# wwood/CoverM

Measured on NVIDIA H100. Metric: reads/sec `coverm contig` (mean+trimmed_mean+covered_fraction), higher is better.
Workload: dtype i32

## Files before the change

coverm_b200/csrc/cmb_k2.cuh:

```cuda
#pragma once
#include "cmb_k2_slots.cuh"

struct K2Args {
  const uint32_t* off_span;
  const uint32_t* len;
  const uint32_t* chunk_first;
  const int32_t* carry_in;
  cmb_contig_stats* rows;
  uint32_t tid_begin, n_local, n_chunks, excl;
  int32_t* arena;
  const uint32_t* word_off;
  const uint16_t* buckets;
  uint32_t* span_bits;
  uint32_t* load_stats;
  const uint64_t* bin_base;
  uint32_t* bins;
  uint64_t pool_cap;
  uint32_t* bin_hi;
  uint32_t* error_flags;
};

#ifndef CMB_K2_DENSE_SPANS
#define CMB_K2_DENSE_SPANS 160
#endif
constexpr uint32_t K2_DENSE_SPANS = CMB_K2_DENSE_SPANS;
static_assert(K2_STAGES >= 2, "a round's rows are requested one round before it is reduced");
static_assert(K2_CHUNK_SPANS == CHUNK_SPANS && K2_WARPS == 8, "a chunk is 8 bitmap words of 32 spans");

constexpr uint32_t K2_ROUND = 32;
constexpr uint32_t K2_BUF_BYTES = K2_ROUND * 128;
constexpr uint32_t K2_BOX_ROWS = K2_ROUND;
constexpr uint32_t K2_STAGE_CODES = 1024;
constexpr uint32_t K2_STAGE_BYTES = K2_STAGE_CODES * 2;
template <bool BUCKETS>
__host__ __device__ constexpr uint32_t k2_warp_bytes() { return BUCKETS ? K2_BUF_BYTES + K2_STAGES * K2_STAGE_BYTES : K2_STAGES * K2_BUF_BYTES; }
constexpr uint32_t K2_SMEM_MISC = K2_WARPS * K2_STAGES * 8  +
                                  K2_WARPS * 128 ;
template <bool BUCKETS>
__host__ __device__ constexpr uint32_t k2_smem_bytes() { return K2_WARPS * k2_warp_bytes<BUCKETS>() + K2_SMEM_MISC; }
static_assert(k2_warp_bytes<true>() % 1024 == 0 && k2_warp_bytes<false>() % 1024 == 0, "round buffers are whole swizzle atoms");

__device__ __forceinline__ uint32_t k2_rounds(uint32_t pop, bool dense) { return dense ? CHUNK_SPANS / K2_ROUND : (pop + K2_ROUND - 1) / K2_ROUND; }

template <bool HIST, bool CLEAN, bool BUCKETS>
__global__ void __launch_bounds__(K2_THREADS, CMB_K2_MINBLOCKS) k2_scan_reduce(const __grid_constant__ CUtensorMap tmap, const K2Args a) {
  extern __shared__ __align__(1024) uint8_t smem[];
  const uint32_t lane = threadIdx.x & 31, warp = threadIdx.x >> 5;
  constexpr uint32_t RING = K2_WARPS * k2_warp_bytes<BUCKETS>();
  uint8_t* ring = smem + warp * k2_warp_bytes<BUCKETS>();
  uint64_t* bars = reinterpret_cast<uint64_t*>(smem + RING) + warp * K2_STAGES;
  uint32_t* words = reinterpret_cast<uint32_t*>(smem + RING + K2_WARPS * K2_STAGES * 8) + warp * 32;
  uint32_t(&fw)[8] = *reinterpret_cast<uint32_t(*)[8]>(words);
  uint32_t(&w)[8] = *reinterpret_cast<uint32_t(*)[8]>(words + 8);
  uint32_t* wo = words + 16;

  const bool hist = HIST && __ldg(a.bin_base + a.n_local) <= a.pool_cap;
  if (HIST && !hist && blockIdx.x == 0 && threadIdx.x == 0) atomicOr(a.error_flags, ERR_CAPACITY);

  const uint32_t W = gridDim.x * K2_WARPS, g = blockIdx.x * K2_WARPS + warp;
  auto load_word = [&](uint32_t ck) -> uint32_t { return ck < a.n_chunks && lane < K2_WARPS ? a.span_bits[ck * K2_WARPS + lane] : 0u; };
  auto load_off = [&](uint32_t ck) -> uint32_t { return BUCKETS && ck < a.n_chunks && lane <= K2_WARPS ? __ldg(a.word_off + ck * K2_WARPS + lane) : 0u; };
  auto spread = [&](uint32_t word, uint32_t* to, uint32_t off = 0, uint32_t* to_off = nullptr) -> uint32_t {
    __syncwarp();
    if (lane < K2_WARPS) to[lane] = word;
    if (to_off && lane <= K2_WARPS) to_off[lane] = off;
    __syncwarp();
    return __reduce_add_sync(FULL, __popc(word));
  };

  if (lane == 0) {
    for (uint32_t s = 0; s < K2_STAGES; ++s) mbar_init(smem_u32(bars + s), 1);
    fence_barrier_init();
  }
  if (BUCKETS)
    for (uint32_t u = lane; u < K2_BUF_BYTES / 16; u += 32) reinterpret_cast<int4*>(ring)[u] = make_int4(0, 0, 0, 0);
  __syncwarp();

  uint32_t fk = g, fr = 0, fpop = 0;
  bool fdense = false;
  uint32_t f_word = load_word(fk);
  uint32_t f_off = load_off(fk), fo = 0;
  uint32_t n_loaded = 0, n_dense = 0, n_events = 0;
  auto f_enter = [&]() {
    for (; fk < a.n_chunks; fk += W) {
      const uint32_t word = f_word;
      f_word = load_word(fk + W);
      fo = f_off;
      f_off = load_off(fk + W);
      fpop = spread(word, fw);
      fdense = fpop >= K2_DENSE_SPANS;
      fr = 0;
      if (k2_rounds(fpop, fdense)) {
        n_loaded += fdense ? CHUNK_SPANS : fpop;
        n_dense += fdense;
        return;
      }
    }
  };
  auto fill = [&](uint32_t fi) {
    if (fk < a.n_chunks) {
      uint8_t* buf = ring + (fi % K2_STAGES) * K2_BUF_BYTES;
      const uint32_t bar = smem_u32(bars + fi % K2_STAGES);
      if constexpr (BUCKETS) {
        uint32_t wf, wl;
        k2_round_words(fw, fdense ? CHUNK_SPANS : fpop, fdense, fr, wf, wl);
        const uint32_t b0 = __shfl_sync(FULL, fo, wf), b1 = __shfl_sync(FULL, fo, wl + 1);
        const uint32_t base = b0 & ~7u, units = min((b1 - base + 7) / 8, K2_STAGE_CODES / 8);
        uint8_t* stg = ring + K2_BUF_BYTES + (fi % K2_STAGES) * K2_STAGE_BYTES;
        const int4* src = reinterpret_cast<const int4*>(a.buckets + base);
        for (uint32_t u = lane; u < units; u += 32) cp_async_16(smem_u32(stg + u * 16), src + u);
        n_events += b1 - b0;
      } else if (fdense) {
        if (lane == 0) {
          fence_proxy_async_smem();
          mbar_arrive_expect_tx(bar, K2_BUF_BYTES);
          tma_load_2d(smem_u32(buf), &tmap, 0, (int32_t)(fk * CHUNK_ROWS + fr * K2_BOX_ROWS), bar);
        }
      } else {
        const uint32_t n = min(K2_ROUND, fpop - fr * K2_ROUND);
        const uint32_t sp = k2_slot_span(fw, fr * K2_ROUND + lane, false);
        const uint32_t q = lane >> 3, unit = lane & 7;
        const int4* src = reinterpret_cast<const int4*>(a.arena + (uint64_t)fk * CHUNK) + unit;
        for (uint32_t r0 = 0; r0 < n; r0 += 4) {
          const uint32_t row = r0 + q;
          const uint32_t rsp = __shfl_sync(FULL, sp, row & 31);
          if (row < n) cp_async_16(smem_u32(buf + row * 128 + ((unit ^ (row & 7)) << 4)), src + rsp * (SPAN / 4));
        }
        if (lane == 0) mbar_arrive(bar);
      }
      if (++fr == k2_rounds(fpop, fdense)) {
        fk += W;
        f_enter();
      }
    }
    cp_async_commit();
  };
  f_enter();
  for (uint32_t p = 0; p + 1 < K2_STAGES; ++p) fill(p);

  const uint32_t E = a.excl;
  auto flush = [&](uint32_t c, uint32_t sf, uint32_t sw, uint64_t sd, uint32_t top) {
    cmb_contig_stats* rowp = a.rows + a.tid_begin + c;
    if (sf) atomicAdd((unsigned long long*)&rowp->covered_full, (unsigned long long)sf);
    if (sw) atomicAdd((unsigned long long*)&rowp->covered_window, (unsigned long long)sw);
    if (sd) atomicAdd((unsigned long long*)&rowp->sum_depth_window, (unsigned long long)sd);
    if (top) atomicMax(a.bin_hi + c, top);
  };
  auto bin_add = [&](uint64_t bin0, uint64_t bin1, int depth, uint32_t cnt, uint32_t& top) {
    if (depth < 0 || (uint64_t)depth >= bin1 - bin0) {
      atomicOr(a.error_flags, ERR_INTERNAL);
      return;
    }
    atomicAdd(a.bins + bin0 + (uint32_t)depth, cnt);
    top = max(top, (uint32_t)depth);
  };

  uint32_t c_word = load_word(g), c_off = load_off(g);
  uint32_t n_cf = 0, n_cl = 0;
  int n_cin = 0;
  if (g < a.n_chunks) {
    n_cf = __ldg(a.chunk_first + g);
    n_cl = __ldg(a.chunk_first + g + 1);
    n_cin = __ldg(a.carry_in + g);
  }
  uint32_t i = 0;
  for (uint32_t k = g; k < a.n_chunks; k += W) {
    const uint32_t word = c_word, off = c_off, cf = n_cf, cl = n_cl;
    const int cin = n_cin;
    c_word = load_word(k + W);
    c_off = load_off(k + W);
    if (k + W < a.n_chunks) {
      n_cf = __ldg(a.chunk_first + k + W);
      n_cl = __ldg(a.chunk_first + k + W + 1);
      n_cin = __ldg(a.carry_in + k + W);
    }
    const uint32_t pop = spread(word, w, off, BUCKETS ? wo : nullptr);
    const bool dense = pop >= K2_DENSE_SPANS;
    const uint32_t nr = k2_rounds(pop, dense), nslots = dense ? CHUNK_SPANS : pop;
    const uint32_t span0 = k * CHUNK_SPANS;
    uint32_t pc = cf, c_first = 0xffffffffu;
    int pd = cin;
    for (uint32_t r = 0; r < nr; ++r, ++i) {
      __syncwarp();
      fill(i + K2_STAGES - 1);
      const uint32_t j = r * K2_ROUND + lane;
      const bool valid = j < nslots;
      const uint32_t s = k2_slot_span(w, j, dense), sn = k2_slot_span(w, j + 1, dense);
      uint32_t c = 0xffffffffu, cstart = 0;
      K2Win win{0u, 0u, 0u};
      uint64_t bin0 = 0, bin1 = 0;
      if (valid) {
        uint32_t lo = cf, hi = cl;
        while (lo < hi) {
          const uint32_t mid = (lo + hi + 1) >> 1;
          if (__ldg(a.off_span + mid) <= span0 + s) lo = mid;
          else hi = mid - 1;
        }
        c = lo;
        cstart = __ldg(a.off_span + c);
        win = k2_window(__ldg(a.len + c), E);
        if (hist) {
          bin0 = __ldg(a.bin_base + c);
          bin1 = __ldg(a.bin_base + c + 1);
        }
      }
      const uint32_t st = i % K2_STAGES;
      if (!BUCKETS) mbar_wait(smem_u32(bars + st), (i / K2_STAGES) & 1);
      cp_async_wait<K2_STAGES - 1>();
      __syncwarp();
      uint8_t* rows = BUCKETS ? ring : ring + st * K2_BUF_BYTES;
      if (BUCKETS) {
        const uint32_t wf = __shfl_sync(FULL, s, 0) / 32, wl = __shfl_sync(FULL, s, min(nslots - r * K2_ROUND, K2_ROUND) - 1) / 32;
        const uint32_t base = wo[wf] & ~7u;
        const uint16_t* stg = reinterpret_cast<const uint16_t*>(ring + K2_BUF_BYTES + st * K2_STAGE_BYTES);
        k2_round_events(
            w, wo, dense, r, wf, wl, lane, 32,
            [&](uint32_t p) { return p - base < K2_STAGE_CODES ? (uint32_t)stg[p - base] : (uint32_t)__ldg(a.buckets + p); },
            [&](uint32_t rw, uint32_t e, int d) {
              atomicAdd(reinterpret_cast<int*>(rows + rw * 128 + (((e >> 2) ^ (rw & 7)) << 4) + ((e & 3) << 2)), d);
            });
        __syncwarp();
      }
      uint8_t* row = rows + lane * 128;
      int total = 0;
      uint32_t ev = 0;
      if (valid) {
#pragma unroll
        for (uint32_t u = 0; u < SPAN / 4; ++u) {
          const int4 v = *reinterpret_cast<const int4*>(row + ((u ^ (lane & 7)) << 4));
          const uint32_t e4 = (v.x != 0 ? 1u : 0u) | (v.y != 0 ? 2u : 0u) | (v.z != 0 ? 4u : 0u) | (v.w != 0 ? 8u : 0u);
          total += (v.x + v.y) + (v.z + v.w);
          ev |= e4 << (4 * u);
          if constexpr (!BUCKETS && CLEAN)
            if (e4) reinterpret_cast<int4*>(a.arena + (uint64_t)(span0 + s) * SPAN)[u] = make_int4(0, 0, 0, 0);
        }
      }
      int incl = total;
#pragma unroll
      for (uint32_t d = 1; d < 32; d <<= 1) {
        const int ov = __shfl_up_sync(FULL, incl, d);
        const uint32_t oc = __shfl_up_sync(FULL, c, d);
        if (lane >= d && oc == c) incl += ov;
      }
      const int depth = incl - total + (c == pc ? pd : 0);
      const uint32_t rel = (span0 + s - cstart) * SPAN;
      const uint32_t from = j == 0 && c == cf ? (span0 - cstart) * SPAN : rel;
      const uint32_t to = rel + (sn - s) * SPAN;
      K2Acc acc{0u, 0u, 0ull};
      uint32_t top = 0;
      int out = 0;
      if (valid)
        out = k2_slot_runs(
            acc, win, depth, ev, rel, from, to,
            [&](uint32_t e) { return *reinterpret_cast<const int*>(row + (((e >> 2) ^ (lane & 7)) << 4) + ((e & 3) << 2)); },
            [&](int d, uint32_t n) {
              if (hist) bin_add(bin0, bin1, d, n, top);
            });
      if (BUCKETS)
#pragma unroll
        for (uint32_t u = 0; u < SPAN / 4; ++u)
          if (ev >> (4 * u) & 15u) *reinterpret_cast<int4*>(row + ((u ^ (lane & 7)) << 4)) = make_int4(0, 0, 0, 0);
      pc = __shfl_sync(FULL, c, 31);
      pd = __shfl_sync(FULL, out, 31);
      if (r == 0) c_first = __shfl_sync(FULL, c, 0);
      uint32_t sf = acc.cov_full, sw = acc.cov_win;
      uint64_t sd = acc.sum_win;
#pragma unroll
      for (uint32_t d = 1; d < 32; d <<= 1) {
        const uint32_t of = __shfl_down_sync(FULL, sf, d), ow = __shfl_down_sync(FULL, sw, d);
        const uint64_t od = __shfl_down_sync(FULL, sd, d);
        const uint32_t ot = HIST ? __shfl_down_sync(FULL, top, d) : 0u;
        const uint32_t oc = __shfl_down_sync(FULL, c, d);
        if (lane + d < 32 && oc == c) {
          sf += of;
          sw += ow;
          sd += od;
          top = max(top, ot);
        }
      }
      const uint32_t prev_c = __shfl_up_sync(FULL, c, 1);
      if (valid && (lane == 0 || prev_c != c)) flush(c, sf, sw, sd, top);
    }
    if (lane == 0 && cin != 0 && c_first != cf) {
      const uint32_t cstart = __ldg(a.off_span + cf);
      const K2Win win = k2_window(__ldg(a.len + cf), E);
      const uint32_t s0 = k2_slot_span(w, 0, dense);
      K2Acc acc{0u, 0u, 0ull};
      uint32_t top = 0;
      const uint32_t nw = k2_close_run(acc, win, cin, (span0 - cstart) * SPAN, (span0 + s0 - cstart) * SPAN);
      if (hist && nw) bin_add(__ldg(a.bin_base + cf), __ldg(a.bin_base + cf + 1), cin, nw, top);
      flush(cf, acc.cov_full, acc.cov_win, acc.sum_win, top);
    }
    if (CLEAN && word) a.span_bits[k * K2_WARPS + lane] = 0;
  }
  if (lane == 0 && n_loaded) {
    atomicAdd(a.load_stats + 0, n_loaded);
    atomicAdd(a.load_stats + 1, n_dense);
    if (BUCKETS) atomicAdd(a.load_stats + 2, n_events);
  }
}
```

coverm_b200/csrc/cmb_k2_slots.cuh:

```cuda
#pragma once
#include <stdint.h>

#ifdef __CUDACC__
#define K2_HD __host__ __device__ __forceinline__
#else
#define K2_HD inline
#endif

constexpr uint32_t K2_CHUNK_SPANS = 256;

K2_HD uint32_t k2_popc(uint32_t x) {
#ifdef __CUDA_ARCH__
  return __popc(x);
#else
  return (uint32_t)__builtin_popcount(x);
#endif
}

K2_HD uint32_t k2_low_bit(uint32_t x) {
#ifdef __CUDA_ARCH__
  return (uint32_t)__ffs((int)x) - 1u;
#else
  return (uint32_t)__builtin_ctz(x);
#endif
}

K2_HD uint32_t k2_nth_bit(uint32_t x, uint32_t n) {
  uint32_t pos = 0;
#pragma unroll
  for (uint32_t w = 16; w; w >>= 1) {
    const uint32_t lo = k2_popc(x & ((1u << w) - 1u));
    if (n >= lo) {
      n -= lo;
      x >>= w;
      pos += w;
    }
  }
  return pos;
}

K2_HD uint32_t k2_slot_span(const uint32_t (&w)[8], uint32_t j, bool dense) {
  if (dense) return j < K2_CHUNK_SPANS ? j : K2_CHUNK_SPANS;
  uint32_t base = 0, word = 0, rem = j;
  bool found = false;
#pragma unroll
  for (uint32_t q = 0; q < 8; ++q) {
    const uint32_t p = k2_popc(w[q]);
    if (!found) {
      if (rem < p) {
        found = true;
        base = 32 * q;
        word = w[q];
      } else {
        rem -= p;
      }
    }
  }
  return found ? base + k2_nth_bit(word, rem) : K2_CHUNK_SPANS;
}


K2_HD void k2_round_words(const uint32_t (&w)[8], uint32_t nslots, bool dense, uint32_t r, uint32_t& wf, uint32_t& wl) {
  const uint32_t j1 = r * 32 + 31 < nslots ? r * 32 + 31 : nslots - 1;
  wf = k2_slot_span(w, r * 32, dense) / 32;
  wl = k2_slot_span(w, j1, dense) / 32;
}

K2_HD uint32_t k2_bucket_row(const uint32_t (&w)[8], bool dense, uint32_t r, uint32_t q, uint32_t before, uint32_t code) {
  const uint32_t b = (code & 1023u) / 32u;
  if (dense) return q * 32 + b - r * 32;
  return before + k2_popc(w[q] & ((1u << b) - 1u)) - r * 32;
}

template <class Code, class Add>
K2_HD void k2_round_events(const uint32_t (&w)[8], const uint32_t* wo, bool dense, uint32_t r, uint32_t wf, uint32_t wl,
                           uint32_t p0, uint32_t step, Code code, Add add) {
  uint32_t q = wf, before = 0;
  for (uint32_t x = 0; x < wf; ++x) before += k2_popc(w[x]);
  const uint32_t p1 = wo[wl + 1];
  for (uint32_t p = wo[wf] + p0; p < p1; p += step) {
    while (q < wl && wo[q + 1] <= p) before += k2_popc(w[q++]);
    const uint32_t c = code(p);
    const uint32_t row = k2_bucket_row(w, dense, r, q, before, c);
    if (row < 32) add(row, c & 31u, (c >> 10) & 1u ? -1 : 1);
  }
}

struct K2Win {
  uint32_t L, w0, w1;
};
K2_HD K2Win k2_window(uint32_t L, uint32_t E) {
  K2Win w{L, 0u, 0u};
  if (2ull * E < L) {
    w.w0 = E;
    w.w1 = L - E;
  }
  return w;
}

struct K2Acc {
  uint32_t cov_full, cov_win;
  uint64_t sum_win;
};

K2_HD uint32_t k2_close_run(K2Acc& a, const K2Win& w, int depth, uint32_t from, uint32_t to) {
  const uint32_t nc = (to < w.L ? to : w.L) - (from < w.L ? from : w.L);
  const uint32_t t1 = to < w.w0 ? w.w0 : (to > w.w1 ? w.w1 : to), f1 = from < w.w0 ? w.w0 : (from > w.w1 ? w.w1 : from);
  const uint32_t nw = t1 - f1;
  if (depth > 0) {
    a.cov_full += nc;
    a.cov_win += nw;
  }
  a.sum_win += (uint64_t)(int64_t)depth * nw;
  return nw;
}

template <class Delta, class Hist>
K2_HD int k2_slot_runs(K2Acc& a, const K2Win& w, int depth, uint32_t ev, uint32_t rel, uint32_t from, uint32_t to, Delta delta,
                       Hist hist) {
  while (ev) {
    const uint32_t j = k2_low_bit(ev);
    ev &= ev - 1;
    const uint32_t nw = k2_close_run(a, w, depth, from, rel + j);
    if (nw && depth != 0) hist(depth, nw);
    depth += delta(j);
    from = rel + j;
  }
  const uint32_t nw = k2_close_run(a, w, depth, from, to);
  if (nw && depth != 0) hist(depth, nw);
  return depth;
}
```

Baseline: 4.583 billion.

## Precompute per-chunk slot-to-span tables and cache chunk contig metadata in smem

Each chunk's span bitmap is expanded once per warp into a shared-memory slot→span byte table plus per-word prefix counts. Slot lookups then become table reads instead of repeated popcount/nth-bit searches in fill, reduce and event decoding. For chunks with fewer than 16 contigs, contig start, length and bin bases are also staged in shared memory, so the contig search becomes a fixed binary search over smem rather than global loads. The cost is extra shared memory per warp, which may reduce occupancy, plus extra work and warp syncs in spread.

```diff
diff --git a/coverm_b200/csrc/cmb_k2.cuh b/coverm_b200/csrc/cmb_k2.cuh
--- a/coverm_b200/csrc/cmb_k2.cuh
+++ b/coverm_b200/csrc/cmb_k2.cuh
@@ -34,8 +34,21 @@
 constexpr uint32_t K2_STAGE_BYTES = K2_STAGE_CODES * 2;
 template <bool BUCKETS>
 __host__ __device__ constexpr uint32_t k2_warp_bytes() { return BUCKETS ? K2_BUF_BYTES + K2_STAGES * K2_STAGE_BYTES : K2_STAGES * K2_BUF_BYTES; }
+constexpr uint32_t K2_CHUNK_CONTIGS = 16;
+struct K2ChunkContigs {
+  uint64_t bin[K2_CHUNK_CONTIGS + 1];
+  uint32_t start[K2_CHUNK_CONTIGS];
+  uint32_t len[K2_CHUNK_CONTIGS];
+};
+struct K2WarpTables {
+  K2ChunkContigs ct;
+  uint8_t span[2][K2_CHUNK_SPANS];
+  uint8_t pre[2][8];
+};
+static_assert(sizeof(K2WarpTables) % 8 == 0, "the contig tables hold u64 bins");
 constexpr uint32_t K2_SMEM_MISC = K2_WARPS * K2_STAGES * 8  +
-                                  K2_WARPS * 128 ;
+                                  K2_WARPS * 128  +
+                                  K2_WARPS * sizeof(K2WarpTables);
 template <bool BUCKETS>
 __host__ __device__ constexpr uint32_t k2_smem_bytes() { return K2_WARPS * k2_warp_bytes<BUCKETS>() + K2_SMEM_MISC; }
 static_assert(k2_warp_bytes<true>() % 1024 == 0 && k2_warp_bytes<false>() % 1024 == 0, "round buffers are whole swizzle atoms");
@@ -50,9 +63,9 @@
   uint8_t* ring = smem + warp * k2_warp_bytes<BUCKETS>();
   uint64_t* bars = reinterpret_cast<uint64_t*>(smem + RING) + warp * K2_STAGES;
   uint32_t* words = reinterpret_cast<uint32_t*>(smem + RING + K2_WARPS * K2_STAGES * 8) + warp * 32;
-  uint32_t(&fw)[8] = *reinterpret_cast<uint32_t(*)[8]>(words);
   uint32_t(&w)[8] = *reinterpret_cast<uint32_t(*)[8]>(words + 8);
   uint32_t* wo = words + 16;
+  K2WarpTables& tb = reinterpret_cast<K2WarpTables*>(smem + RING + K2_WARPS * K2_STAGES * 8 + K2_WARPS * 128)[warp];
 
   const bool hist = HIST && __ldg(a.bin_base + a.n_local) <= a.pool_cap;
   if (HIST && !hist && blockIdx.x == 0 && threadIdx.x == 0) atomicOr(a.error_flags, ERR_CAPACITY);
@@ -60,12 +73,23 @@
   const uint32_t W = gridDim.x * K2_WARPS, g = blockIdx.x * K2_WARPS + warp;
   auto load_word = [&](uint32_t ck) -> uint32_t { return ck < a.n_chunks && lane < K2_WARPS ? a.span_bits[ck * K2_WARPS + lane] : 0u; };
   auto load_off = [&](uint32_t ck) -> uint32_t { return BUCKETS && ck < a.n_chunks && lane <= K2_WARPS ? __ldg(a.word_off + ck * K2_WARPS + lane) : 0u; };
-  auto spread = [&](uint32_t word, uint32_t* to, uint32_t off = 0, uint32_t* to_off = nullptr) -> uint32_t {
+  auto spread = [&](uint32_t word, uint32_t* to, uint32_t t, uint32_t off = 0, uint32_t* to_off = nullptr) -> uint32_t {
     __syncwarp();
-    if (lane < K2_WARPS) to[lane] = word;
+    if (to && lane < K2_WARPS) to[lane] = word;
     if (to_off && lane <= K2_WARPS) to_off[lane] = off;
+    const uint32_t pop = __reduce_add_sync(FULL, __popc(word));
+    const uint32_t mw = pop >= K2_DENSE_SPANS && lane < K2_WARPS ? ~0u : word;
+    uint32_t before = __popc(mw);
+#pragma unroll
+    for (uint32_t d = 1; d < K2_WARPS; d <<= 1) {
+      const uint32_t o = __shfl_up_sync(FULL, before, d);
+      if (lane >= d) before += o;
+    }
+    before -= __popc(mw);
+    if (lane < K2_WARPS) tb.pre[t][lane] = (uint8_t)before;
+    k2_span_table_lane(__shfl_sync(FULL, mw, lane / 4), __shfl_sync(FULL, before, lane / 4), lane, tb.span[t]);
     __syncwarp();
-    return __reduce_add_sync(FULL, __popc(word));
+    return pop;
   };
 
   if (lane == 0) {
@@ -76,8 +100,7 @@
     for (uint32_t u = lane; u < K2_BUF_BYTES / 16; u += 32) reinterpret_cast<int4*>(ring)[u] = make_int4(0, 0, 0, 0);
   __syncwarp();
 
-  uint32_t fk = g, fr = 0, fpop = 0;
-  bool fdense = false;
+  uint32_t fk = g, fr = 0, fns = 0;
   uint32_t f_word = load_word(fk);
   uint32_t f_off = load_off(fk), fo = 0;
   uint32_t n_loaded = 0, n_dense = 0, n_events = 0;
@@ -87,12 +110,12 @@
       f_word = load_word(fk + W);
       fo = f_off;
       f_off = load_off(fk + W);
-      fpop = spread(word, fw);
-      fdense = fpop >= K2_DENSE_SPANS;
+      const uint32_t pop = spread(word, nullptr, 0);
+      fns = pop >= K2_DENSE_SPANS ? CHUNK_SPANS : pop;
       fr = 0;
-      if (k2_rounds(fpop, fdense)) {
-        n_loaded += fdense ? CHUNK_SPANS : fpop;
-        n_dense += fdense;
+      if (fns) {
+        n_loaded += fns;
+        n_dense += pop >= K2_DENSE_SPANS;
         return;
       }
     }
@@ -103,22 +126,22 @@
       const uint32_t bar = smem_u32(bars + fi % K2_STAGES);
       if constexpr (BUCKETS) {
         uint32_t wf, wl;
-        k2_round_words(fw, fdense ? CHUNK_SPANS : fpop, fdense, fr, wf, wl);
+        k2_round_words(tb.span[0], fns, fr, wf, wl);
         const uint32_t b0 = __shfl_sync(FULL, fo, wf), b1 = __shfl_sync(FULL, fo, wl + 1);
         const uint32_t base = b0 & ~7u, units = min((b1 - base + 7) / 8, K2_STAGE_CODES / 8);
         uint8_t* stg = ring + K2_BUF_BYTES + (fi % K2_STAGES) * K2_STAGE_BYTES;
         const int4* src = reinterpret_cast<const int4*>(a.buckets + base);
         for (uint32_t u = lane; u < units; u += 32) cp_async_16(smem_u32(stg + u * 16), src + u);
         n_events += b1 - b0;
-      } else if (fdense) {
+      } else if (fns >= K2_DENSE_SPANS) {
         if (lane == 0) {
           fence_proxy_async_smem();
           mbar_arrive_expect_tx(bar, K2_BUF_BYTES);
           tma_load_2d(smem_u32(buf), &tmap, 0, (int32_t)(fk * CHUNK_ROWS + fr * K2_BOX_ROWS), bar);
         }
       } else {
-        const uint32_t n = min(K2_ROUND, fpop - fr * K2_ROUND);
-        const uint32_t sp = k2_slot_span(fw, fr * K2_ROUND + lane, false);
+        const uint32_t n = min(K2_ROUND, fns - fr * K2_ROUND);
+        const uint32_t jf = fr * K2_ROUND + lane, sp = jf < fns ? tb.span[0][jf] : 0u;
         const uint32_t q = lane >> 3, unit = lane & 7;
         const int4* src = reinterpret_cast<const int4*>(a.arena + (uint64_t)fk * CHUNK) + unit;
         for (uint32_t r0 = 0; r0 < n; r0 += 4) {
@@ -128,7 +151,7 @@
         }
         if (lane == 0) mbar_arrive(bar);
       }
-      if (++fr == k2_rounds(fpop, fdense)) {
+      if (++fr == (fns + K2_ROUND - 1) / K2_ROUND) {
         fk += W;
         f_enter();
       }
@@ -174,7 +197,21 @@
       n_cl = __ldg(a.chunk_first + k + W + 1);
       n_cin = __ldg(a.carry_in + k + W);
     }
-    const uint32_t pop = spread(word, w, off, BUCKETS ? wo : nullptr);
+    const bool tabled = BUCKETS && cl - cf < K2_CHUNK_CONTIGS;
+    uint32_t t_start = 0, t_len = 0;
+    uint64_t t_bin = 0;
+    if (tabled && lane <= cl - cf) {
+      t_start = __ldg(a.off_span + cf + lane);
+      t_len = __ldg(a.len + cf + lane);
+    }
+    if (HIST && tabled && lane <= cl - cf + 1) t_bin = __ldg(a.bin_base + cf + lane);
+    const uint32_t pop = spread(word, w, 1, off, BUCKETS ? wo : nullptr);
+    if (tabled && lane <= cl - cf) {
+      tb.ct.start[lane] = t_start;
+      tb.ct.len[lane] = t_len;
+    }
+    if (HIST && tabled && lane <= cl - cf + 1) tb.ct.bin[lane] = t_bin;
+    __syncwarp();
     const bool dense = pop >= K2_DENSE_SPANS;
     const uint32_t nr = k2_rounds(pop, dense), nslots = dense ? CHUNK_SPANS : pop;
     const uint32_t span0 = k * CHUNK_SPANS;
@@ -185,11 +222,23 @@
       fill(i + K2_STAGES - 1);
       const uint32_t j = r * K2_ROUND + lane;
       const bool valid = j < nslots;
-      const uint32_t s = k2_slot_span(w, j, dense), sn = k2_slot_span(w, j + 1, dense);
+      const uint32_t s = valid ? tb.span[1][j] : CHUNK_SPANS, sn = j + 1 < nslots ? tb.span[1][j + 1] : CHUNK_SPANS;
       uint32_t c = 0xffffffffu, cstart = 0;
       K2Win win{0u, 0u, 0u};
       uint64_t bin0 = 0, bin1 = 0;
-      if (valid) {
+      if (valid && tabled) {
+        uint32_t t = 0;
+#pragma unroll
+        for (uint32_t h = K2_CHUNK_CONTIGS / 2; h; h >>= 1)
+          if (t + h <= cl - cf && tb.ct.start[t + h] <= span0 + s) t += h;
+        c = cf + t;
+        cstart = tb.ct.start[t];
+        win = k2_window(tb.ct.len[t], E);
+        if (hist) {
+          bin0 = tb.ct.bin[t];
+          bin1 = tb.ct.bin[t + 1];
+        }
+      } else if (valid) {
         uint32_t lo = cf, hi = cl;
         while (lo < hi) {
           const uint32_t mid = (lo + hi + 1) >> 1;
@@ -214,7 +263,7 @@
         const uint32_t base = wo[wf] & ~7u;
         const uint16_t* stg = reinterpret_cast<const uint16_t*>(ring + K2_BUF_BYTES + st * K2_STAGE_BYTES);
         k2_round_events(
-            w, wo, dense, r, wf, wl, lane, 32,
+            w, tb.pre[1], wo, dense, r, wf, wl, lane, 32,
             [&](uint32_t p) { return p - base < K2_STAGE_CODES ? (uint32_t)stg[p - base] : (uint32_t)__ldg(a.buckets + p); },
             [&](uint32_t rw, uint32_t e, int d) {
               atomicAdd(reinterpret_cast<int*>(rows + rw * 128 + (((e >> 2) ^ (rw & 7)) << 4) + ((e & 3) << 2)), d);
@@ -282,13 +331,14 @@
       if (valid && (lane == 0 || prev_c != c)) flush(c, sf, sw, sd, top);
     }
     if (lane == 0 && cin != 0 && c_first != cf) {
-      const uint32_t cstart = __ldg(a.off_span + cf);
-      const K2Win win = k2_window(__ldg(a.len + cf), E);
-      const uint32_t s0 = k2_slot_span(w, 0, dense);
+      const uint32_t cstart = tabled ? tb.ct.start[0] : __ldg(a.off_span + cf);
+      const K2Win win = k2_window(tabled ? tb.ct.len[0] : __ldg(a.len + cf), E);
+      const uint32_t s0 = nslots ? tb.span[1][0] : CHUNK_SPANS;
       K2Acc acc{0u, 0u, 0ull};
       uint32_t top = 0;
       const uint32_t nw = k2_close_run(acc, win, cin, (span0 - cstart) * SPAN, (span0 + s0 - cstart) * SPAN);
-      if (hist && nw) bin_add(__ldg(a.bin_base + cf), __ldg(a.bin_base + cf + 1), cin, nw, top);
+      if (hist && nw)
+        bin_add(tabled ? tb.ct.bin[0] : __ldg(a.bin_base + cf), tabled ? tb.ct.bin[1] : __ldg(a.bin_base + cf + 1), cin, nw, top);
       flush(cf, acc.cov_full, acc.cov_win, acc.sum_win, top);
     }
     if (CLEAN && word) a.span_bits[k * K2_WARPS + lane] = 0;
diff --git a/coverm_b200/csrc/cmb_k2_slots.cuh b/coverm_b200/csrc/cmb_k2_slots.cuh
--- a/coverm_b200/csrc/cmb_k2_slots.cuh
+++ b/coverm_b200/csrc/cmb_k2_slots.cuh
@@ -59,11 +59,25 @@
   return found ? base + k2_nth_bit(word, rem) : K2_CHUNK_SPANS;
 }
 
+K2_HD void k2_span_table_lane(uint32_t word, uint32_t before, uint32_t lane, uint8_t* span) {
+  const uint32_t q = lane / 4, sh = (lane % 4) * 8;
+  uint32_t m = (word >> sh) & 255u, j = before + k2_popc(word & ((1u << sh) - 1u));
+  while (m) {
+    span[j++] = (uint8_t)(32 * q + sh + k2_low_bit(m));
+    m &= m - 1;
+  }
+}
+
 
 K2_HD void k2_round_words(const uint32_t (&w)[8], uint32_t nslots, bool dense, uint32_t r, uint32_t& wf, uint32_t& wl) {
   const uint32_t j1 = r * 32 + 31 < nslots ? r * 32 + 31 : nslots - 1;
   wf = k2_slot_span(w, r * 32, dense) / 32;
   wl = k2_slot_span(w, j1, dense) / 32;
+}
+K2_HD void k2_round_words(const uint8_t* span, uint32_t nslots, uint32_t r, uint32_t& wf, uint32_t& wl) {
+  const uint32_t j1 = r * 32 + 31 < nslots ? r * 32 + 31 : nslots - 1;
+  wf = span[r * 32] / 32u;
+  wl = span[j1] / 32u;
 }
 
 K2_HD uint32_t k2_bucket_row(const uint32_t (&w)[8], bool dense, uint32_t r, uint32_t q, uint32_t before, uint32_t code) {
@@ -73,17 +87,23 @@
 }
 
 template <class Code, class Add>
-K2_HD void k2_round_events(const uint32_t (&w)[8], const uint32_t* wo, bool dense, uint32_t r, uint32_t wf, uint32_t wl,
-                           uint32_t p0, uint32_t step, Code code, Add add) {
-  uint32_t q = wf, before = 0;
-  for (uint32_t x = 0; x < wf; ++x) before += k2_popc(w[x]);
+K2_HD void k2_round_events(const uint32_t (&w)[8], const uint8_t* pre, const uint32_t* wo, bool dense, uint32_t r, uint32_t wf,
+                           uint32_t wl, uint32_t p0, uint32_t step, Code code, Add add) {
+  uint32_t q = wf, before = pre[wf];
   const uint32_t p1 = wo[wl + 1];
   for (uint32_t p = wo[wf] + p0; p < p1; p += step) {
-    while (q < wl && wo[q + 1] <= p) before += k2_popc(w[q++]);
+    while (q < wl && wo[q + 1] <= p) before = pre[++q];
     const uint32_t c = code(p);
     const uint32_t row = k2_bucket_row(w, dense, r, q, before, c);
     if (row < 32) add(row, c & 31u, (c >> 10) & 1u ? -1 : 1);
   }
+}
+template <class Code, class Add>
+K2_HD void k2_round_events(const uint32_t (&w)[8], const uint32_t* wo, bool dense, uint32_t r, uint32_t wf, uint32_t wl,
+                           uint32_t p0, uint32_t step, Code code, Add add) {
+  uint8_t pre[8];
+  for (uint32_t q = 0, before = 0; q < 8; before += k2_popc(w[q++])) pre[q] = (uint8_t)before;
+  k2_round_events(w, pre, wo, dense, r, wf, wl, p0, step, code, add);
 }
 
 struct K2Win {
```

Measured after the change: 5.457 billion (median of 6 runs). 19.1% higher.
